# SebastianBitsch/SRGAN-ST

Hardware: AMD Instinct MI355X
Metric: HR images/sec (96px x4, B=16/GPU) G+D+ST-loss step (higher is better)
Workload: dtype f32; 1 GPU; srgan_x4_hr96_b16_G+D+ST-loss step: adv+mse+st, D updated every step (train.py:116-164; BASELINE metric); global_batch=16, hr=96, lr=24, parallelism=dp1, hip_graph=True, d_update_interval=1, d_sr_forward=run: all three discriminator forwards of train.py:136,155,158

## Files before the change

include/srganst.h:

```cpp
#ifndef SRGANST_H
#define SRGANST_H
#include <stdint.h>
#ifdef __cplusplus
extern "C" {
#endif

const char* sst_last_error(void);
int sst_version(void);
const char* sst_arch(void);
int sst_clear_error(void);
int sst_reload_env(void);

int sst_st_loss_workspace(int B, int H, int W, int64_t* partial_floats);
int sst_st_loss_fwd(const float* sr, const float* gt, float* loss, float* gS, float* partials,
                    unsigned* counter, int B, int H, int W, float sigma, float rho, int normalize,
                    void* stream);
int sst_st_loss_bwd(const float* sr, const float* gS, float* dsr, const float* scale_dev,
                    float scale_host, int accumulate, int B, int H, int W, float sigma, float rho,
                    void* stream);
int sst_st_maps_workspace(int B, int H, int W, int64_t* tile_floats);
int sst_st_maps(const float* x, const float* gt, float* Sx, float* Sgt, float* Fx, float* Fgt, float* d, float* tile_sums,
                int B, int H, int W, float sigma, float rho, int normalize, void* stream);
int sst_st_pixel_loss_fwd(const float* sr, const float* gt, float* loss, float* gS, float* partials, unsigned* counter,
                          float* pix_loss, float* pix_partials, int pix_mode, int B, int H, int W, float sigma, float rho,
                          int normalize, void* stream);
int sst_st_pixel_loss_bwd(const float* sr, const float* gt, const float* gS, float* dsr, const float* scale_dev, float scale_host,
                          float pix_weight, int pix_mode, int accumulate, int B, int H, int W, float sigma, float rho,
                          void* stream);

int64_t sst_conv_packed_floats(int Cout, int Cin, int ksize);
int sst_conv_pack(const float* w, float* wp, int Cout, int Cin, int ksize, int mode, void* stream);
int sst_conv_pack_multi(const void* jobs, int njobs, int total_blocks, void* stream);
int sst_conv_mtiles(int B, int Ho, int Wo);
int sst_conv_stat_tiles(int B, int H, int W, int Cin, int Cout, int ksize, int stride);
const char* sst_conv_kernel_name(int B, int H, int W, int Cin, int Cout, int ksize, int stride, int out_mode, int fused_in);
const char* sst_conv_wgrad_kernel_name(int B, int H, int W, int Cin, int Cout, int ksize, int stride, int njobs);
long sst_debug_big_tile_launches(void);
long sst_debug_band_launches(void);
long sst_debug_wgrad_band_launches(void);
int sst_debug_mfma_peak(float* out, int blocks, int iters, void* stream);
int sst_debug_bf16x3(const float* A, const float* B, float* C32, float* C3, int K, int mode, int blocks, void* stream);
int sst_debug_stamp(unsigned long long* out, int slot, void* stream);
int sst_conv_fwd(const float* x, const float* wp, float* y, float* y_pre, const float* bias,
                 const float* in_scale, const float* in_shift, const float* in_slope,
                 float in_slope_const, int in_act, const float* residual, float* stats,
                 float* stats_cnt, int out_mode, int B, int H, int W, int Cin, int Cout, int ksize,
                 int stride, void* stream);
int sst_conv_pipe_supported(int B, int H, int W, int Cin, int Cout, int ksize, int stride);
int sst_conv_pipe_stat_tiles(int B, int H, int W, int Cin, int Cout, int ksize, int stride);
int64_t sst_conv_pipe_ws_floats(int B, int H, int W, int Cin, int Cout, int ksize, int stride);
int sst_conv_pipe_fwd(const float* x, const float* wp, float* y, const float* bias, const float* in_scale,
                      const float* in_shift, const float* in_slope, float in_slope_const, int in_act, float* stats,
                      float* stats_cnt, const float* epi_y, const float* epi_scale, const float* epi_shift,
                      const float* epi_slope, float epi_slope_const, int epi_act, float* epi_partial, float* ws, int B,
                      int H, int W, int Cin, int Cout, int ksize, int stride, void* stream);
int sst_conv_pipe_groups_ok(int B, int H, int W, int Cin, int Cout, int ksize, int stride, int grp_images);
int sst_conv_pipe_fwd_grp(const float* x, const float* wp, float* y, const float* bias, const float* in_scale,
                          const float* in_shift, const float* in_slope, float in_slope_const, int in_act, float* stats,
                          float* stats_cnt, const float* epi_y, const float* epi_scale, const float* epi_shift,
                          const float* epi_slope, float epi_slope_const, int epi_act, float* epi_partial, float* ws, int B,
                          int H, int W, int Cin, int Cout, int ksize, int stride, int grp_images, void* stream);
int sst_conv_ns_supported(int B, int H, int W, int Cin, int Cout, int ksize, int stride, int out_mode);
int sst_conv_ns_fwd(const float* x, const float* wp, float* y, const float* bias, const float* in_scale,
                    const float* in_shift, const float* in_slope, float in_slope_const, int in_act, float* stats,
                    float* stats_cnt, const float* epi_y, const float* epi_scale, const float* epi_shift,
                    const float* epi_slope, float epi_slope_const, int epi_act, float* epi_partial, int B, int H, int W,
                    int Cin, int Cout, int ksize, int stride, int out_mode, int grp_images, void* stream);
int sst_conv_s2_dgrad_pipe_supported(int B, int H, int W, int Cin, int Cout);
int64_t sst_conv_s2_dgrad_pipe_ws_floats(int B, int H, int W, int Cin, int Cout);
int sst_conv_s2_dgrad_pipe(const float* dy, const float* wp, float* dx, float* ws, int B, int H, int W, int Cin, int Cout,
                           void* stream);
int sst_conv_s2_dgrad_pipe_stat_tiles(int B, int H, int W, int Cin, int Cout);
int sst_conv_s2_dgrad_pipe_bwdstats(const float* dy, const float* wp, float* dx, float* ws, const float* epi_y,
                                    const float* epi_scale, const float* epi_shift, const float* epi_slope,
                                    float epi_slope_const, int epi_act, float* epi_partial, int B, int H, int W, int Cin,
                                    int Cout, void* stream);
int sst_conv_s2_dgrad_pipe_groups_ok(int B, int H, int W, int Cin, int Cout, int grp_images);
int sst_conv_s2_dgrad_pipe_bwdstats_grp(const float* dy, const float* wp, float* dx, float* ws, const float* epi_y,
                                    const float* epi_scale, const float* epi_shift, const float* epi_slope,
                                    float epi_slope_const, int epi_act, float* epi_partial, int B, int H, int W, int Cin,
                                    int Cout, int grp_images, void* stream);
int sst_conv_dgrad_bwdstats(const float* x, const float* wp, float* y, const float* residual, const float* epi_y,
                            const float* epi_scale, const float* epi_shift, const float* epi_slope,
// ... 184 lines not shown
```

srgan-st_amd/csrc/conv_pipe.hip:

```cpp
#include "conv_common.h"
#include <cstdlib>
#include <type_traits>
#include "conv_epilogue.h"

int sst_conv_band_rows(int B, int H, int W, int Cin, int Cout, int ksize, int stride);

namespace {

constexpr int PIPE_RING = 9;

struct PipeArgs {
  const float* x;
  const float* wp;
  float* y;
  const float* bias;
  const float* in_scale; const float* in_shift; const float* in_slope; float in_slope_const; int in_act;
  float* stats; float* stats_cnt;
  const float* epi_y; const float* epi_scale; const float* epi_shift; const float* epi_slope;
  float epi_slope_const; int epi_act; float* epi_partial;
  float* ws;
  int B, H, W, Cin, Cout, Ho, Wo;
  int R;
  int tiles_x, n_mt, nfc, total_tiles, ncb, ksplit, cb_per, units;
#ifdef SST_PIPE_ABLATE
  int dbg;
#endif
  int gB, grows;
};

template <int S, int TW, int MODE>
struct PipeGeom {
  static constexpr int TH = 32 / TW;
  static constexpr int NB = TW == 2 ? 3 : 1;
  static constexpr int KSPAN = MODE ? 2 : 3;
  static constexpr int PW = (TW - 1) * S + KSPAN;
  static constexpr int PR = (TH - 1) * S + KSPAN + NB;
  static constexpr int NP = PW * PR;
  static constexpr int NU = (NP + 15) / 16;
  static constexpr int PS = 20;
  static constexpr int WAVE_FLOATS = NP * PS;
  static constexpr int NACC = MODE ? 4 : 1;
  static constexpr int NPAIR = MODE ? 2 : 1;
  static constexpr int SCRATCH = NPAIR * 4 * 32 * 33;
};
constexpr int S2D_CLS[9] = {0, 1, 1, 2, 2, 3, 3, 3, 3};
constexpr int S2D_TAP[9] = {0, 0, 1, 0, 1, 0, 1, 2, 3};

struct Stage {
  int b0, rem0, ix0, c0;
  int gin;
  const float* w;
};

#define PIPE_GLOAD(dst, voff, sbase) \
  asm volatile("s_nop 4\n\tglobal_load_dwordx4 %0, %1, %2" : "=v"(dst) : "v"(voff), "s"(sbase))
#define PIPE_WAIT(reg, n) asm volatile("s_waitcnt vmcnt(%1)" : "+v"(reg) : "n"(n))

__device__ __forceinline__ float half_sum(float t) {
  auto ror = [](float x, auto ctrl) {
    return __builtin_bit_cast(float, __builtin_amdgcn_update_dpp(0, __builtin_bit_cast(int, x), decltype(ctrl)::value, 0xf, 0xf, false));
  };
  t += ror(t, std::integral_constant<int, 0x128>{});
  t += ror(t, std::integral_constant<int, 0x124>{});
  t += ror(t, std::integral_constant<int, 0x122>{});
  t += ror(t, std::integral_constant<int, 0x121>{});
  t += __shfl_xor(t, 16, 64);
  return t;
}

template <int TW, int MODE = 0>
__device__ __forceinline__ void pipe_epilogue(const PipeArgs& a, float v[4], int r0, int ox0, int c0, int mt, int lane, bool first,
                                              int cls = 0) {
  constexpr int TH = 32 / TW;
  const int px = lane & 31;
  const int r = r0 + px / TW, ox = ox0 + px % TW;
  const bool pix_ok = r < a.R && ox < a.Wo;
  size_t obase;
  if (MODE) {
    obase = ((size_t)(2 * r + (cls >> 1)) * (2 * a.Wo) + 2 * ox + (cls & 1)) * a.Cout + c0;
    if (pix_ok) *reinterpret_cast<f32x4*>(a.y + obase) = f32x4{v[0], v[1], v[2], v[3]};
  }
  if (!MODE && a.bias) {
    const f32x4 bv = *reinterpret_cast<const f32x4*>(a.bias + c0);
#pragma unroll
    for (int j = 0; j < 4; ++j) v[j] += bv[j];
  }
  if (!MODE) {
    obase = ((size_t)r * a.Wo + ox) * a.Cout + c0;
    if (pix_ok) *reinterpret_cast<f32x4*>(a.y + obase) = f32x4{v[0], v[1], v[2], v[3]};
// ... 17 lines not shown
    }
  }
  if (a.epi_partial) {
    const float eslope = a.epi_slope ? a.epi_slope[0] : a.epi_slope_const;
    f32x4 yv = {0.f, 0.f, 0.f, 0.f}, es = {1.f, 1.f, 1.f, 1.f}, eh = {0.f, 0.f, 0.f, 0.f};
    if (pix_ok) yv = *reinterpret_cast<const f32x4*>(a.epi_y + obase);
    if (a.epi_scale) {
      const int ge = a.gB ? (r0 / a.grows) * a.Cout : 0;
      es = *reinterpret_cast<const f32x4*>(a.epi_scale + ge + c0);
      eh = *reinterpret_cast<const f32x4*>(a.epi_shift + ge + c0);
    }
    f32x4 q[3];
#pragma unroll
    for (int j = 0; j < 4; ++j) {
      const float g = pix_ok ? v[j] : 0.f;
      const float z = a.epi_scale ? fmaf(yv[j], es[j], eh[j]) : yv[j];
      float gz = g, q2 = 0.f;
      if (a.epi_act) {
        q2 = g * fminf(z, 0.f);
        gz = z > 0.f ? g : g * eslope;
      }
      q[0][j] = half_sum(gz);
      q[1][j] = half_sum(gz * yv[j]);
      q[2][j] = half_sum(q2);
    }
    if (px == 0) {
      const size_t prow = MODE ? (size_t)mt * 4 + cls : (size_t)mt;
#pragma unroll
      for (int k = 0; k < 3; ++k) *reinterpret_cast<f32x4*>(a.epi_partial + (prow * 3 + k) * a.Cout + c0) = q[k];
    }
  }
}

template <int S, int TW, int MODE, bool MS>
__global__ __launch_bounds__(CONV_NT, (S == 1 && MODE == 0 ? 3 : 2)) void conv_pipe_kernel(PipeArgs a) {
  using G = PipeGeom<S, TW, MODE>;
  constexpr int NACC = G::NACC, NPAIR = G::NPAIR;
  constexpr int PW = G::PW, NP = G::NP, NU = G::NU, NB = G::NB;
  constexpr int PS = G::PS;
  __shared__ __attribute__((aligned(16))) float patch[4 * G::WAVE_FLOATS];
  __shared__ __attribute__((aligned(16))) float scratch[G::SCRATCH];
  const int tid = threadIdx.x, wave = __builtin_amdgcn_readfirstlane(tid >> 6), lane = tid & 63;
  const int li = lane & 31, lh = lane >> 5;
  const int nwg = gridDim.x;
  const int HV = a.H + 1;
  const float slope = a.in_slope ? a.in_slope[0] : a.in_slope_const;
  const int c4 = wave * 16 + (lane & 3) * 4;
  const int p0 = lane >> 2;
  float* const lds = patch + wave * G::WAVE_FLOATS;

  int q = blockIdx.x;
  if (q >= a.units) return;
  int mt, nf, r0, ox0, oy0, cb, cb_end;
  Stage cur, nxt;
  auto decode = [&](int qq, int& mt_, int& nf_, int& ksi_, int& r0_, int& ox0_, int& b0_, int& oy0_) {
    mt_ = qq % a.n_mt;
    const int rest = qq / a.n_mt;
    nf_ = rest % a.nfc;
    ksi_ = rest / a.nfc;
    const int ty = mt_ / a.tiles_x, tx = mt_ - ty * a.tiles_x;
    r0_ = ty * G::TH;
    ox0_ = tx * TW;
    b0_ = r0_ / a.Ho;
    oy0_ = r0_ - b0_ * a.Ho;
  };
  auto make_stage = [&](int b0_, int oy0_, int ox0_, int nf_, int cb_) {
    Stage s;
    s.b0 = b0_;
    s.rem0 = oy0_ * S;
    s.ix0 = ox0_ * S - (MODE ? 0 : 1);
    s.c0 = cb_ * CB;
    s.gin = a.gB ? (b0_ / a.gB) * a.Cin : 0;
    s.w = a.wp + ((size_t)(nf_ * a.ncb + cb_) * 9 * 8) * 256 + wave * 512;
    return s;
  };
  int ksi, b0;
  decode(q, mt, nf, ksi, r0, ox0, b0, oy0);
  cb = ksi * a.cb_per;
  cb_end = cb + a.cb_per;
  cur = make_stage(b0, oy0, ox0, nf, cb);

  constexpr int NS = NU + 2;
  f32x4 sv[NU];
  unsigned okmask = 0;
  f32x4 ssc, ssh;
  const float* sc_base = a.in_scale ? a.in_scale : a.x;
  const float* sh_base = a.in_scale ? a.in_shift : a.x;
  unsigned boffs[MS ? NU : 1];
  auto stage_load = [&](const Stage& s, bool same_tile) {
#ifdef SST_PIPE_ABLATE
    if (a.dbg & 4) return;
#endif
    if (MS && same_tile) {
#pragma unroll
      for (int u = 0; u < NU; ++u) {
        boffs[u] += CB * 4u;
        PIPE_GLOAD(sv[u], boffs[u], a.x);
      }
    } else {
      okmask = 0;
#pragma unroll
      for (int u = 0; u < NU; ++u) {
        const int p = p0 + 16 * u;
        const int pr = p / PW, pc = p - pr * PW;
        int rr = s.rem0 + pr, b = s.b0;
#pragma unroll
        for (int k = 0; k <= NB; ++k) {
          const bool wrap = rr >= HV;
          rr -= wrap ? HV : 0;
          b += wrap ? 1 : 0;
        }
        const int iy = MODE ? rr : rr - 1, ix = s.ix0 + pc;
        const bool ok = p < NP && (MODE ? rr < a.H : rr >= 1) && b < a.B && (unsigned)ix < (unsigned)a.W;
        const int off = ((b * a.H + iy) * a.W + ix) * a.Cin + s.c0 + c4;
        const unsigned boff = (ok ? (unsigned)off : (unsigned)c4) * 4u;
        if (MS) boffs[u] = boff;
        PIPE_GLOAD(sv[u], boff, a.x);
        okmask |= ok ? (1u << u) : 0u;
      }
    }
    const unsigned coff = (unsigned)(a.in_scale ? s.gin + s.c0 + c4 : c4) * 4u;
    PIPE_GLOAD(ssc, coff, sc_base);
    PIPE_GLOAD(ssh, coff, sh_base);
  };
  auto stage_store = [&]() {
#ifdef SST_PIPE_ABLATE
    if (a.dbg & 1) return;
#endif
#pragma unroll
    for (int u = 0; u < NU; ++u) {
      const int p = p0 + 16 * u;
      if (p >= NP) continue;
      f32x4 t = sv[u];
      if (a.in_scale) {
#pragma unroll
        for (int j = 0; j < 4; ++j) t[j] = fmaf(t[j], ssc[j], ssh[j]);
      }
      if (a.in_act == ACT_SLOPE) {
#pragma unroll
        for (int j = 0; j < 4; ++j) t[j] = t[j] > 0.f ? t[j] : t[j] * slope;
      }
      if (!((okmask >> u) & 1u)) t = f32x4{0.f, 0.f, 0.f, 0.f};
      *reinterpret_cast<f32x4*>(&lds[p * PS + (lane & 3) * 4]) = t;
    }
  };

  auto lane_base = [&](int oy0_) {
    const int tr = li / TW, tc = li - tr * TW;
    int cross = 0;
#pragma unroll
    for (int k = 1; k <= NB; ++k) cross += (oy0_ + tr >= k * a.Ho) ? 1 : 0;
    return ((S * tr + cross) * PW + tc * S) * PS + 4 * lh;
  };
  int a_base = lane_base(oy0);

  f32x4 ring[PIPE_RING];
  const unsigned wlane = lane * 16u;
#define PIPE_WCHUNK(dst, w, i) PIPE_GLOAD(dst, wlane, (w) + (((i) >> 1) * 8 + ((i) & 1)) * 256)

#pragma unroll
  for (int i = 0; i < PIPE_RING; ++i) PIPE_WCHUNK(ring[i], cur.w, i);
  stage_load(cur, false);
  asm volatile("s_waitcnt vmcnt(0)" ::: "memory");
  __builtin_amdgcn_sched_barrier(0);
  stage_store();

  f32x16 acc[NACC];
#pragma unroll
  for (int k = 0; k < NACC; ++k)
#pragma unroll
    for (int r = 0; r < 16; ++r) acc[k][r] = 0.f;

  for (;;) {
    const bool unit_end = cb + 1 == cb_end;
    int n_q = q, n_mt = mt, n_nf = nf, n_r0 = r0, n_ox0 = ox0, n_oy0 = oy0, n_cb = cb + 1, n_cb_end = cb_end;
    bool more = true;
    if (unit_end) {
      n_q = q + nwg;
      more = n_q < a.units;
      if (more) {
        int n_ksi, n_b0;
        decode(n_q, n_mt, n_nf, n_ksi, n_r0, n_ox0, n_b0, n_oy0);
        n_cb = n_ksi * a.cb_per;
        n_cb_end = n_cb + a.cb_per;
        nxt = make_stage(n_b0, n_oy0, n_ox0, n_nf, n_cb);
      } else {
        nxt = cur;
      }
    } else {
      nxt = cur;
      nxt.c0 += CB;
      nxt.w += (size_t)9 * 8 * 256;
    }

    {
      const float* ab = lds + a_base;
      f32x4 av = *reinterpret_cast<const f32x4*>(ab);
      __builtin_amdgcn_sched_barrier(0);
#pragma unroll
      for (int i = 0; i < 18; ++i) {
        f32x4 an = av;
        if (i + 1 < 18) {
          const int t = (i + 1) >> 1;
          const int ntx = MODE ? 1 + (S2D_CLS[t] & 1) : 3, tt = MODE ? S2D_TAP[t] : t;
          an = *reinterpret_cast<const f32x4*>(ab + ((tt / ntx) * PW + (tt % ntx)) * PS + ((i + 1) & 1) * 8);
        }
        if (i == 0 || i >= 10) PIPE_WAIT(ring[i % PIPE_RING], 8); else PIPE_WAIT(ring[i % PIPE_RING], 8 + NS);
        const f32x4 bv = ring[i % PIPE_RING];
        constexpr int dummy_ = 0;
        (void)dummy_;
        const int ai = MODE ? S2D_CLS[i >> 1] : 0;
#ifdef SST_PIPE_ABLATE
        if (!(a.dbg & 16))
#endif
#pragma unroll
        for (int j = 0; j < 4; ++j) acc[ai] = __builtin_amdgcn_mfma_f32_32x32x2f32(av[j], bv[j], acc[ai], 0, 0, 0);
#ifdef SST_PIPE_ABLATE
        if (a.dbg & 8) { PIPE_GLOAD(ring[i % PIPE_RING], wlane, a.wp); } else
#endif
        if (i + PIPE_RING < 18) PIPE_WCHUNK(ring[i % PIPE_RING], cur.w, i + PIPE_RING);
        else PIPE_WCHUNK(ring[i % PIPE_RING], nxt.w, i + PIPE_RING - 18);
        if (i == 0) stage_load(nxt, !unit_end);
        av = an;
        __builtin_amdgcn_sched_barrier(0);
      }
    }
#ifdef SST_PIPE_ABLATE
    if (unit_end && (a.dbg & 2)) {
      if (acc[0][0] == 12345.f) a.y[0] = acc[0][0];
      if (!more) return;
      a_base = lane_base(n_oy0);
    } else
#endif
    if (unit_end) {
      const int cl = 8 * wave + 4 * lh;
#pragma unroll
      for (int k0 = 0; k0 < NACC; k0 += NPAIR) {
        __syncthreads();
#pragma unroll
        for (int k = 0; k < NPAIR; ++k)
#pragma unroll
          for (int r = 0; r < 16; ++r) {
            const int row = (r & 3) + 8 * (r >> 2) + 4 * lh;
            scratch[((k * 4 + wave) * 32 + row) * 33 + li] = acc[k0 + k][r];
            acc[k0 + k][r] = 0.f;
          }
        __syncthreads();
#pragma unroll
        for (int k = 0; k < NPAIR; ++k) {
          float v[4];
#pragma unroll
          for (int j = 0; j < 4; ++j) {
            float t = scratch[((k * 4 + 0) * 32 + li) * 33 + cl + j];
            t += scratch[((k * 4 + 1) * 32 + li) * 33 + cl + j];
            t += scratch[((k * 4 + 2) * 32 + li) * 33 + cl + j];
            t += scratch[((k * 4 + 3) * 32 + li) * 33 + cl + j];
            v[j] = t;
          }
          if (a.ksplit > 1) {
            const int tile = nf * a.n_mt + mt;
            const int part = cb / a.cb_per;
            *reinterpret_cast<f32x4*>(a.ws + (((size_t)part * a.total_tiles + tile) * NACC + k0 + k) * 1024 + li * 32 + cl) =
                f32x4{v[0], v[1], v[2], v[3]};
          } else {
            pipe_epilogue<TW, MODE>(a, v, r0, ox0, nf * 32 + cl, mt, lane, nf == 0 && wave == 0, k0 + k);
          }
        }
      }
      if (!more) return;
      a_base = lane_base(n_oy0);
    }
    stage_store();
    q = n_q; mt = n_mt; nf = n_nf; r0 = n_r0; ox0 = n_ox0; oy0 = n_oy0; cb = n_cb; cb_end = n_cb_end;
    cur = nxt;
  }
}

template <int TW, int MODE>
__global__ __launch_bounds__(CONV_NT) void pipe_reduce_kernel(PipeArgs a) {
  constexpr int NACC = MODE ? 4 : 1;
  const int tid = threadIdx.x, wave = tid >> 6, lane = tid & 63;
  const int tile = blockIdx.x / NACC, cls = blockIdx.x - tile * NACC;
  const int nf = tile / a.n_mt, mt = tile - nf * a.n_mt;
  const int ty = mt / a.tiles_x, tx = mt - ty * a.tiles_x;
  const int li = lane & 31, cl = 8 * wave + 4 * (lane >> 5);
  const size_t slab = (size_t)a.total_tiles * NACC * 1024;
  const float* src = a.ws + ((size_t)tile * NACC + cls) * 1024 + li * 32 + cl;
  f32x4 s = *reinterpret_cast<const f32x4*>(src);
  for (int k = 1; k < a.ksplit; ++k) {
    const f32x4 t = *reinterpret_cast<const f32x4*>(src + k * slab);
#pragma unroll
    for (int j = 0; j < 4; ++j) s[j] += t[j];
  }
  float v[4] = {s[0], s[1], s[2], s[3]};
  pipe_epilogue<TW, MODE>(a, v, ty * (32 / TW), tx * TW, nf * 32 + cl, mt, lane, nf == 0 && wave == 0, cls);
}

struct PipePlan {
  int tw;
  int ksplit, n_mt, tiles_x, nfc, ncb;
};

PipePlan pipe_plan(int B, int H, int W, int Cin, int Cout, int ksize, int stride) {
  PipePlan pl{};
  if (ksize != 3 || (stride != 1 && stride != 2) || (Cin % 64) || (Cout % 32) || B <= 0) return pl;
  if (stride == 2 && ((H | W) & 1)) return pl;
  if (Cout <= 64 && sst_conv_band_rows(B, H, W, Cin, Cout, ksize, stride)) return pl;
  const int Ho = (H - 1) / stride + 1, Wo = (W - 1) / stride + 1;
  int tw = 0;
  if (Wo % 8 == 0 && Ho >= 3) tw = 8;
  else if (Wo % 4 == 0 && Ho >= 7) tw = 4;
  else if (Wo % 2 == 0 && Ho >= 5) tw = 2;
  if (!tw) return pl;
  const int th = 32 / tw;
  pl.tiles_x = Wo / tw;
  pl.n_mt = pl.tiles_x * ((B * Ho + th - 1) / th);
  pl.nfc = Cout / 32;
  pl.ncb = Cin / 64;
  const long tiles = (long)pl.n_mt * pl.nfc;
  int maxks = 1;
  while (maxks < 4 && pl.ncb % (maxks * 2) == 0) maxks *= 2;
  if (tiles * maxks < 256) return pl;
  int ks = 1;
  while (tiles * ks < 1024 && ks < maxks) ks *= 2;
  pl.ksplit = ks;
  pl.tw = tw;
  return pl;
}

constexpr int PIPE_CUS = 256;

}

SST_API int sst_conv_pipe_supported(int B, int H, int W, int Cin, int Cout, int ksize, int stride) {
  return pipe_plan(B, H, W, Cin, Cout, ksize, stride).tw;
}
SST_API int sst_conv_pipe_stat_tiles(int B, int H, int W, int Cin, int Cout, int ksize, int stride) {
  return pipe_plan(B, H, W, Cin, Cout, ksize, stride).n_mt;
}
SST_API int64_t sst_conv_pipe_ws_floats(int B, int H, int W, int Cin, int Cout, int ksize, int stride) {
  const PipePlan pl = pipe_plan(B, H, W, Cin, Cout, ksize, stride);
  return (pl.tw && pl.ksplit > 1) ? (int64_t)pl.ksplit * pl.n_mt * pl.nfc * 1024 : 0;
}

SST_API int sst_conv_pipe_groups_ok(int B, int H, int W, int Cin, int Cout, int ksize, int stride, int grp_images) {
  const PipePlan pl = pipe_plan(B, H, W, Cin, Cout, ksize, stride);
  if (!pl.tw || grp_images <= 0 || B % grp_images) return 0;
  const int Ho = (H - 1) / stride + 1;
  return (grp_images * Ho) % (32 / pl.tw) == 0;
}

SST_API int sst_conv_pipe_fwd_grp(const float* x, const float* wp, float* y, const float* bias, const float* in_scale,
                                  const float* in_shift, const float* in_slope, float in_slope_const, int in_act, float* stats,
                                  float* stats_cnt, const float* epi_y, const float* epi_scale, const float* epi_shift,
                                  const float* epi_slope, float epi_slope_const, int epi_act, float* epi_partial, float* ws, int B,
                                  int H, int W, int Cin, int Cout, int ksize, int stride, int grp_images, void* stream) {
  SST_REQUIRE(x && wp && y, "sst_conv_pipe_fwd: null pointer");
  const PipePlan pl = pipe_plan(B, H, W, Cin, Cout, ksize, stride);
  SST_REQUIRE(grp_images == 0 || grp_images == B || sst_conv_pipe_groups_ok(B, H, W, Cin, Cout, ksize, stride, grp_images),
              "sst_conv_pipe_fwd: coefficient groups of %d images do not end on tile boundaries (B=%d H=%d W=%d stride=%d)", grp_images, B,
              H, W, stride);
  SST_REQUIRE(pl.tw, "sst_conv_pipe_fwd: shape B=%d H=%d W=%d Cin=%d Cout=%d k=%d stride=%d is not taken by the pipelined kernel", B,
              H, W, Cin, Cout, ksize, stride);
  SST_REQUIRE((in_scale == nullptr) == (in_shift == nullptr), "sst_conv_pipe_fwd: in_scale/in_shift must come together");
  SST_REQUIRE(!stats || stats_cnt, "sst_conv_pipe_fwd: stats needs stats_cnt");
  SST_REQUIRE(!epi_partial || (epi_y && !stats && ((epi_scale == nullptr) == (epi_shift == nullptr))),
              "sst_conv_pipe_fwd: backward partials need epi_y and exclude forward stats");
  SST_REQUIRE(pl.ksplit == 1 || ws, "sst_conv_pipe_fwd: this shape splits K over workgroups and needs the workspace");
  SST_REQUIRE((int64_t)B * H * W * Cin < (1ll << 29), "sst_conv_pipe_fwd: input too large for 32-bit byte offsets");
  PipeArgs a;
  a.x = x; a.wp = wp; a.y = y; a.bias = bias; a.in_scale = in_scale; a.in_shift = in_shift; a.in_slope = in_slope;
  a.in_slope_const = in_slope_const; a.in_act = in_act; a.stats = stats; a.stats_cnt = stats_cnt;
  a.epi_y = epi_y; a.epi_scale = epi_scale; a.epi_shift = epi_shift; a.epi_slope = epi_slope; a.epi_slope_const = epi_slope_const;
  a.epi_act = epi_act; a.epi_partial = epi_partial; a.ws = ws;
  a.B = B; a.H = H; a.W = W; a.Cin = Cin; a.Cout = Cout;
  a.Ho = (H - 1) / stride + 1; a.Wo = (W - 1) / stride + 1; a.R = B * a.Ho;
  a.tiles_x = pl.tiles_x; a.n_mt = pl.n_mt; a.nfc = pl.nfc; a.total_tiles = pl.n_mt * pl.nfc; a.ncb = pl.ncb;
  a.ksplit = pl.ksplit; a.cb_per = pl.ncb / pl.ksplit; a.units = a.total_tiles * pl.ksplit;
  a.gB = (grp_images > 0 && grp_images < B) ? grp_images : 0;
  a.grows = a.gB * a.Ho;
#ifdef SST_PIPE_ABLATE
  a.dbg = sst_env("SST_PIPE_DBG") ? atoi(sst_env("SST_PIPE_DBG")) : 0;
#endif
  int wg_per_cu = stride == 1 ? 3 : 2;
  if (const char* e = sst_env("SST_PIPE_GPC")) {
    const int v = atoi(e);
    if (v >= 1 && v < wg_per_cu) wg_per_cu = v;
  }
  const int grid = a.units < wg_per_cu * PIPE_CUS ? a.units : wg_per_cu * PIPE_CUS;
  hipStream_t st = sst_stream(stream);
#define SST_PIPE_LAUNCH(S_, TW_)                                                                  \
  do {                                                                                            \
    if (a.cb_per > 1) conv_pipe_kernel<S_, TW_, 0, true><<<grid, CONV_NT, 0, st>>>(a);            \
    else conv_pipe_kernel<S_, TW_, 0, false><<<grid, CONV_NT, 0, st>>>(a);                        \
    SST_LAUNCH_CHECK("conv_pipe_kernel");                                                         \
    if (pl.ksplit > 1) {                                                                          \
      pipe_reduce_kernel<TW_, 0><<<a.total_tiles, CONV_NT, 0, st>>>(a);                           \
      SST_LAUNCH_CHECK("pipe_reduce_kernel");                                                     \
    }                                                                                             \
  } while (0)
  if (stride == 1) {
    if (pl.tw == 8) SST_PIPE_LAUNCH(1, 8); else if (pl.tw == 4) SST_PIPE_LAUNCH(1, 4); else SST_PIPE_LAUNCH(1, 2);
  } else {
    if (pl.tw == 8) SST_PIPE_LAUNCH(2, 8); else if (pl.tw == 4) SST_PIPE_LAUNCH(2, 4); else SST_PIPE_LAUNCH(2, 2);
  }
#undef SST_PIPE_LAUNCH
  return SST_OK;
}

SST_API int sst_conv_pipe_fwd(const float* x, const float* wp, float* y, const float* bias, const float* in_scale,
                              const float* in_shift, const float* in_slope, float in_slope_const, int in_act, float* stats,
                              float* stats_cnt, const float* epi_y, const float* epi_scale, const float* epi_shift,
                              const float* epi_slope, float epi_slope_const, int epi_act, float* epi_partial, float* ws, int B,
                              int H, int W, int Cin, int Cout, int ksize, int stride, void* stream) {
  return sst_conv_pipe_fwd_grp(x, wp, y, bias, in_scale, in_shift, in_slope, in_slope_const, in_act, stats, stats_cnt, epi_y, epi_scale,
                               epi_shift, epi_slope, epi_slope_const, epi_act, epi_partial, ws, B, H, W, Cin, Cout, ksize, stride, 0, stream);
}

int64_t sst_conv_s2_dgrad_pipe_section(int Cout, int Cin);
SST_API int sst_conv_s2_dgrad_pipe_bwdstats_grp(const float* dy, const float* wp, float* dx, float* ws, const float* epi_y,
                                                const float* epi_scale, const float* epi_shift, const float* epi_slope,
                                                float epi_slope_const, int epi_act, float* epi_partial, int B, int H, int W, int Cin,
                                                int Cout, int grp_images, void* stream);

namespace {
PipePlan pipe_plan_s2d(int B, int H, int W, int Cin, int Cout) {
// ... 92 lines not shown
```

srgan-st_amd/srganst/_abi.py:

```python
from __future__ import annotations

import ctypes
import os
from ctypes import c_char_p, c_float, c_int, c_int64, c_void_p, POINTER

_HERE = os.path.dirname(os.path.abspath(__file__))
LIB_PATH = os.environ.get("SST_LIB_PATH") or os.path.join(_HERE, "lib", "libsrganst.so")

P = c_void_p

SIGNATURES = {
    "sst_last_error": (c_char_p, []),
    "sst_version": (c_int, []),
    "sst_arch": (c_char_p, []),
    "sst_clear_error": (c_int, []),
    "sst_reload_env": (c_int, []),
    "sst_st_loss_workspace": (c_int, [c_int, c_int, c_int, POINTER(c_int64)]),
    "sst_st_loss_fwd": (c_int, [P, P, P, P, P, P, c_int, c_int, c_int, c_float, c_float, c_int, P]),
    "sst_st_loss_bwd": (c_int, [P, P, P, P, c_float, c_int, c_int, c_int, c_int, c_float, c_float, P]),
    "sst_st_pixel_loss_fwd": (c_int, [P, P, P, P, P, P, P, P, c_int, c_int, c_int, c_int, c_float, c_float, c_int, P]),
    "sst_st_pixel_loss_bwd": (c_int, [P, P, P, P, P, c_float, c_float, c_int, c_int, c_int, c_int, c_int, c_float, c_float, P]),
    "sst_st_maps_workspace": (c_int, [c_int, c_int, c_int, POINTER(c_int64)]),
    "sst_st_maps": (c_int, [P, P, P, P, P, P, P, P, c_int, c_int, c_int, c_float, c_float, c_int, P]),
    "sst_conv_packed_floats": (c_int64, [c_int, c_int, c_int]),
    "sst_conv_pack": (c_int, [P, P, c_int, c_int, c_int, c_int, P]),
    "sst_conv_pack_multi": (c_int, [P, c_int, c_int, P]),
    "sst_conv_kernel_name": (c_char_p, [c_int, c_int, c_int, c_int, c_int, c_int, c_int, c_int, c_int]),
    "sst_conv_wgrad_kernel_name": (c_char_p, [c_int, c_int, c_int, c_int, c_int, c_int, c_int, c_int]),
    "sst_debug_big_tile_launches": (ctypes.c_long, []),
    "sst_adam_flat": (c_int, [P, P, P, P, c_int64, P, P, c_int, ctypes.c_double, ctypes.c_double, ctypes.c_double,
                            ctypes.c_double, P]),
    "sst_debug_band_launches": (ctypes.c_long, []),
    "sst_debug_wgrad_band_launches": (ctypes.c_long, []),
    "sst_debug_mfma_peak": (c_int, [P, c_int, c_int, P]),
    "sst_debug_bf16x3": (c_int, [P, P, P, P, c_int, c_int, c_int, P]),
    "sst_debug_stamp": (c_int, [P, c_int, P]),
    "sst_conv_mtiles": (c_int, [c_int, c_int, c_int]),
    "sst_conv_stat_tiles": (c_int, [c_int, c_int, c_int, c_int, c_int, c_int, c_int]),
    "sst_conv_fwd": (c_int, [P, P, P, P, P, P, P, P, c_float, c_int, P, P, P, c_int,
                             c_int, c_int, c_int, c_int, c_int, c_int, c_int, P]),
    "sst_conv_pipe_supported": (c_int, [c_int, c_int, c_int, c_int, c_int, c_int, c_int]),
    "sst_conv_pipe_stat_tiles": (c_int, [c_int, c_int, c_int, c_int, c_int, c_int, c_int]),
    "sst_conv_pipe_ws_floats": (c_int64, [c_int, c_int, c_int, c_int, c_int, c_int, c_int]),
    "sst_conv_pipe_fwd": (c_int, [P, P, P, P, P, P, P, c_float, c_int, P, P, P, P, P, P, c_float, c_int, P, P,
                                  c_int, c_int, c_int, c_int, c_int, c_int, c_int, P]),
    "sst_conv_pipe_groups_ok": (c_int, [c_int, c_int, c_int, c_int, c_int, c_int, c_int, c_int]),
    "sst_conv_pipe_fwd_grp": (c_int, [P, P, P, P, P, P, P, c_float, c_int, P, P, P, P, P, P, c_float, c_int, P, P,
                                      c_int, c_int, c_int, c_int, c_int, c_int, c_int, c_int, P]),
    "sst_conv_ns_supported": (c_int, [c_int, c_int, c_int, c_int, c_int, c_int, c_int, c_int]),
    "sst_conv_ns_fwd": (c_int, [P, P, P, P, P, P, P, c_float, c_int, P, P, P, P, P, P, c_float, c_int, P,
                                c_int, c_int, c_int, c_int, c_int, c_int, c_int, c_int, c_int, P]),
    "sst_conv_s2_dgrad_pipe_supported": (c_int, [c_int, c_int, c_int, c_int, c_int]),
    "sst_conv_s2_dgrad_pipe_ws_floats": (c_int64, [c_int, c_int, c_int, c_int, c_int]),
    "sst_conv_s2_dgrad_pipe": (c_int, [P, P, P, P, c_int, c_int, c_int, c_int, c_int, P]),
    "sst_conv_s2_dgrad_pipe_stat_tiles": (c_int, [c_int, c_int, c_int, c_int, c_int]),
    "sst_conv_s2_dgrad_pipe_bwdstats": (c_int, [P, P, P, P, P, P, P, P, c_float, c_int, P, c_int, c_int, c_int, c_int, c_int, P]),
    "sst_conv_s2_dgrad_pipe_groups_ok": (c_int, [c_int, c_int, c_int, c_int, c_int, c_int]),
    "sst_conv_s2_dgrad_pipe_bwdstats_grp": (c_int, [P, P, P, P, P, P, P, P, c_float, c_int, P, c_int, c_int, c_int, c_int, c_int, c_int, P]),
    "sst_conv_acc_supported": (c_int, [c_int, c_int, c_int, c_int, c_int, c_int, c_int]),
    "sst_conv_fwd_acc": (c_int, [P, P, P, P, P, P, P, P, c_float, c_int, P, P, P, c_float, c_float, c_float, P, P, P, P, P, P, P,
                                 c_int, c_int, c_int, c_int, c_int, c_int, c_int, P]),
    "sst_conv_dgrad_fused_acc": (c_int, [P, P, P, P, P, c_float, c_int, P, P, P, P, P, P, P, P, c_float, c_int, P, P, P, P, c_float, P, P, P,
                                         P, c_int, c_int, c_int, c_int, c_int, c_int, c_int, P]),
    "sst_bn_finalize_acc": (c_int, [P, c_int, c_int, c_float, P, P, P, P, P, P, P, P, c_float, c_float, P]),
    "sst_conv_fwd_resin": (c_int, [P, P, P, P, P, P, P, P, P, P, P, c_int, c_int, c_int, c_int, c_int, c_int, P]),
    "sst_conv_dgrad_bwdstats": (c_int, [P, P, P, P, P, P, P, P, c_float, c_int, P, c_int, c_int, c_int, c_int, c_int, c_int, P]),
    "sst_conv_dgrad_fused": (c_int, [P, P, P, P, P, P, P, P, c_float, c_int, P, P, P, P, P, P, P, P, c_float, c_int, P,
                                     c_int, c_int, c_int, c_int, c_int, c_int, P]),
    "sst_conv_wgrad_chunks": (c_int, [c_int, c_int, c_int, c_int, c_int, c_int]),
    "sst_conv_wgrad_chunks2": (c_int, [c_int, c_int, c_int, c_int, c_int, c_int, c_int, c_int]),
    "sst_conv_wgrad": (c_int, [P, P, P, P, P, P, P, c_float, c_int, c_int, c_int, c_int, c_int, c_int,
                               c_int, c_int, c_int, P]),
    "sst_conv_wgrad_groups_ok": (c_int, [c_int, c_int, c_int, c_int, c_int, c_int, c_int, c_int]),
    "sst_conv_wgrad_grp": (c_int, [P, P, P, P, P, P, P, c_float, c_int, c_int, c_int, c_int, c_int, c_int,
                                   c_int, c_int, c_int, c_int, P]),
    "sst_conv_wgrad_grouped": (c_int, [P, c_int, c_int, c_int, c_int, c_int, c_int, c_int, c_int, c_int, P]),
# ... 120 lines not shown
```

Before: 3262 HR images/s.

## Pair adjacent output-channel blocks in stride-2 pipelined conv to reuse input patches

Adds 'pair units' to the stride-2 forward pipelined conv kernel. One workgroup computes two adjacent 32-channel output blocks, sharing the LDS input patch and A operands while streaming two weight rings with a smaller ring depth. A host-side makespan model picks how many channel pairs to form so that fewer, heavier units fill the 256-CU grid better. This trades extra registers and lower occupancy risk, plus a more complex wait and epilogue path, for less input reload and better wave quantization.

Result: no change. 3267 HR images/s, median of 6 (+0.2%).

```diff
diff --git a/include/srganst.h b/include/srganst.h
--- a/include/srganst.h
+++ b/include/srganst.h
@@ -49,6 +49,7 @@
 int sst_conv_pipe_supported(int B, int H, int W, int Cin, int Cout, int ksize, int stride);
 int sst_conv_pipe_stat_tiles(int B, int H, int W, int Cin, int Cout, int ksize, int stride);
 int64_t sst_conv_pipe_ws_floats(int B, int H, int W, int Cin, int Cout, int ksize, int stride);
+int sst_conv_pipe_pair_units(int B, int H, int W, int Cin, int Cout, int ksize, int stride, int* pairs, int* singles);
 int sst_conv_pipe_fwd(const float* x, const float* wp, float* y, const float* bias, const float* in_scale,
                       const float* in_shift, const float* in_slope, float in_slope_const, int in_act, float* stats,
                       float* stats_cnt, const float* epi_y, const float* epi_scale, const float* epi_shift,
diff --git a/srgan-st_amd/csrc/conv_pipe.hip b/srgan-st_amd/csrc/conv_pipe.hip
--- a/srgan-st_amd/csrc/conv_pipe.hip
+++ b/srgan-st_amd/csrc/conv_pipe.hip
@@ -8,6 +8,7 @@
 namespace {
 
 constexpr int PIPE_RING = 9;
+constexpr int PIPE_RING_PAIR = 6;
 
 struct PipeArgs {
   const float* x;
@@ -26,6 +27,7 @@
   int dbg;
 #endif
   int gB, grows;
+  int npair, pair_units;
 };
 
 template <int S, int TW, int MODE>
@@ -55,6 +57,7 @@
 #define PIPE_GLOAD(dst, voff, sbase) \
   asm volatile("s_nop 4\n\tglobal_load_dwordx4 %0, %1, %2" : "=v"(dst) : "v"(voff), "s"(sbase))
 #define PIPE_WAIT(reg, n) asm volatile("s_waitcnt vmcnt(%1)" : "+v"(reg) : "n"(n))
+#define PIPE_WAIT2(reg, reg2, n) asm volatile("s_waitcnt vmcnt(%2)" : "+v"(reg), "+v"(reg2) : "n"(n))
 
 __device__ __forceinline__ float half_sum(float t) {
   auto ror = [](float x, auto ctrl) {
@@ -138,8 +141,9 @@
   }
 }
 
-template <int S, int TW, int MODE, bool MS>
+template <int S, int TW, int MODE, bool MS, bool PAIRS = false>
 __global__ __launch_bounds__(CONV_NT, (S == 1 && MODE == 0 ? 3 : 2)) void conv_pipe_kernel(PipeArgs a) {
+  static_assert(!PAIRS || (S == 2 && MODE == 0), "pair units: stride-2 forward only");
   using G = PipeGeom<S, TW, MODE>;
   constexpr int NACC = G::NACC, NPAIR = G::NPAIR;
   constexpr int PW = G::PW, NP = G::NP, NU = G::NU, NB = G::NB;
@@ -151,19 +155,32 @@
   const int nwg = gridDim.x;
   const int HV = a.H + 1;
   const float slope = a.in_slope ? a.in_slope[0] : a.in_slope_const;
-  const int c4 = wave * 16 + (lane & 3) * 4;
+  const int c4_ = wave * 16 + (lane & 3) * 4;
   const int p0 = lane >> 2;
   float* const lds = patch + wave * G::WAVE_FLOATS;
 
   int q = blockIdx.x;
   if (q >= a.units) return;
   int mt, nf, r0, ox0, oy0, cb, cb_end;
+  bool pair = false;
   Stage cur, nxt;
-  auto decode = [&](int qq, int& mt_, int& nf_, int& ksi_, int& r0_, int& ox0_, int& b0_, int& oy0_) {
-    mt_ = qq % a.n_mt;
-    const int rest = qq / a.n_mt;
-    nf_ = rest % a.nfc;
-    ksi_ = rest / a.nfc;
+  auto decode = [&](int qq, int& mt_, int& nf_, int& ksi_, int& r0_, int& ox0_, int& b0_, int& oy0_, bool& pair_) {
+    if constexpr (PAIRS) {
+      pair_ = qq < a.pair_units;
+      const int slots = pair_ ? a.npair : a.nfc - 2 * a.npair;
+      if (!pair_) qq -= a.pair_units;
+      mt_ = qq % a.n_mt;
+      const int rest = qq / a.n_mt;
+      const int slot = rest % slots;
+      nf_ = pair_ ? 2 * slot : 2 * a.npair + slot;
+      ksi_ = rest / slots;
+    } else {
+      pair_ = false;
+      mt_ = qq % a.n_mt;
+      const int rest = qq / a.n_mt;
+      nf_ = rest % a.nfc;
+      ksi_ = rest / a.nfc;
+    }
     const int ty = mt_ / a.tiles_x, tx = mt_ - ty * a.tiles_x;
     r0_ = ty * G::TH;
     ox0_ = tx * TW;
@@ -181,10 +198,13 @@
     return s;
   };
   int ksi, b0;
-  decode(q, mt, nf, ksi, r0, ox0, b0, oy0);
+  decode(q, mt, nf, ksi, r0, ox0, b0, oy0, pair);
   cb = ksi * a.cb_per;
   cb_end = cb + a.cb_per;
   cur = make_stage(b0, oy0, ox0, nf, cb);
+  const size_t wblk2 = (size_t)a.ncb * 72 * 256;
+  const float* cur_w2 = cur.w + (pair ? wblk2 : 0);
+  const float* nxt_w2 = cur_w2;
 
   constexpr int NS = NU + 2;
   f32x4 sv[NU];
@@ -193,7 +213,7 @@
   const float* sc_base = a.in_scale ? a.in_scale : a.x;
   const float* sh_base = a.in_scale ? a.in_shift : a.x;
   unsigned boffs[MS ? NU : 1];
-  auto stage_load = [&](const Stage& s, bool same_tile) {
+  auto stage_load = [&](const Stage& s, bool same_tile) __attribute__((always_inline)) {
 #ifdef SST_PIPE_ABLATE
     if (a.dbg & 4) return;
 #endif
@@ -205,10 +225,20 @@
       }
     } else {
       okmask = 0;
+      int p0v = p0, c4 = c4_;
+      if constexpr (PAIRS) asm volatile("" : "+v"(p0v), "+v"(c4));
+      int pr_u = p0v / PW, pc_u = p0v - pr_u * PW;
 #pragma unroll
       for (int u = 0; u < NU; ++u) {
-        const int p = p0 + 16 * u;
-        const int pr = p / PW, pc = p - pr * PW;
+        const int p = p0v + 16 * u;
+        int pr, pc;
+        if constexpr (PAIRS) {
+          pr = pr_u; pc = pc_u;
+          pc_u += 16 % PW; pr_u += 16 / PW;
+          if (pc_u >= PW) { pc_u -= PW; ++pr_u; }
+        } else {
+          pr = p / PW; pc = p - pr * PW;
+        }
         int rr = s.rem0 + pr, b = s.b0;
 #pragma unroll
         for (int k = 0; k <= NB; ++k) {
@@ -225,11 +255,11 @@
         okmask |= ok ? (1u << u) : 0u;
       }
     }
-    const unsigned coff = (unsigned)(a.in_scale ? s.gin + s.c0 + c4 : c4) * 4u;
+    const unsigned coff = (unsigned)(a.in_scale ? s.gin + s.c0 + c4_ : c4_) * 4u;
     PIPE_GLOAD(ssc, coff, sc_base);
     PIPE_GLOAD(ssh, coff, sh_base);
   };
-  auto stage_store = [&]() {
+  auto stage_store = [&]() __attribute__((always_inline)) {
 #ifdef SST_PIPE_ABLATE
     if (a.dbg & 1) return;
 #endif
@@ -252,132 +282,117 @@
   };
 
   auto lane_base = [&](int oy0_) {
-    const int tr = li / TW, tc = li - tr * TW;
+    int li_b = li, lh_b = lh;
+    if constexpr (PAIRS) {
+      int lane_b = lane;
+      asm volatile("" : "+v"(lane_b));
+      li_b = lane_b & 31; lh_b = lane_b >> 5;
+    }
+    const int tr = li_b / TW, tc = li_b - tr * TW;
     int cross = 0;
 #pragma unroll
     for (int k = 1; k <= NB; ++k) cross += (oy0_ + tr >= k * a.Ho) ? 1 : 0;
-    return ((S * tr + cross) * PW + tc * S) * PS + 4 * lh;
+    return ((S * tr + cross) * PW + tc * S) * PS + 4 * lh_b;
   };
   int a_base = lane_base(oy0);
 
-  f32x4 ring[PIPE_RING];
+  constexpr int RING = PAIRS ? PIPE_RING_PAIR : PIPE_RING;
+  static_assert(18 % RING == 0, "a stage's 18 chunks must fill the ring a whole number of times");
+  f32x4 ring[RING];
+  f32x4 ring2[PAIRS ? RING : 1];
   const unsigned wlane = lane * 16u;
 #define PIPE_WCHUNK(dst, w, i) PIPE_GLOAD(dst, wlane, (w) + (((i) >> 1) * 8 + ((i) & 1)) * 256)
 
 #pragma unroll
-  for (int i = 0; i < PIPE_RING; ++i) PIPE_WCHUNK(ring[i], cur.w, i);
+  for (int i = 0; i < RING; ++i) PIPE_WCHUNK(ring[i], cur.w, i);
+  if constexpr (PAIRS) {
+    if (pair) {
+#pragma unroll
+      for (int i = 0; i < RING; ++i) PIPE_WCHUNK(ring2[i], cur_w2, i);
+    } else {
+#pragma unroll
+      for (int i = 0; i < RING; ++i) ring2[i] = f32x4{0.f, 0.f, 0.f, 0.f};
+    }
+  }
   stage_load(cur, false);
   asm volatile("s_waitcnt vmcnt(0)" ::: "memory");
   __builtin_amdgcn_sched_barrier(0);
   stage_store();
 
-  f32x16 acc[NACC];
-#pragma unroll
-  for (int k = 0; k < NACC; ++k)
+  constexpr int NACC2 = PAIRS ? 2 : NACC;
+  f32x16 acc[NACC2];
+#pragma unroll
+  for (int k = 0; k < NACC2; ++k)
 #pragma unroll
     for (int r = 0; r < 16; ++r) acc[k][r] = 0.f;
 
   for (;;) {
     const bool unit_end = cb + 1 == cb_end;
     int n_q = q, n_mt = mt, n_nf = nf, n_r0 = r0, n_ox0 = ox0, n_oy0 = oy0, n_cb = cb + 1, n_cb_end = cb_end;
-    bool more = true;
+    bool more = true, n_pair = pair;
     if (unit_end) {
       n_q = q + nwg;
       more = n_q < a.units;
       if (more) {
         int n_ksi, n_b0;
-        decode(n_q, n_mt, n_nf, n_ksi, n_r0, n_ox0, n_b0, n_oy0);
+        decode(n_q, n_mt, n_nf, n_ksi, n_r0, n_ox0, n_b0, n_oy0, n_pair);
         n_cb = n_ksi * a.cb_per;
         n_cb_end = n_cb + a.cb_per;
         nxt = make_stage(n_b0, n_oy0, n_ox0, n_nf, n_cb);
       } else {
         nxt = cur;
       }
+      if constexpr (PAIRS) nxt_w2 = nxt.w + (more && n_pair ? wblk2 : 0);
     } else {
       nxt = cur;
       nxt.c0 += CB;
       nxt.w += (size_t)9 * 8 * 256;
-    }
-
+      if constexpr (PAIRS) nxt_w2 = cur_w2 + (size_t)9 * 8 * 256;
+    }
+
+#define PIPE_SECTION_KLOOP
     {
-      const float* ab = lds + a_base;
-      f32x4 av = *reinterpret_cast<const f32x4*>(ab);
-      __builtin_amdgcn_sched_barrier(0);
-#pragma unroll
-      for (int i = 0; i < 18; ++i) {
-        f32x4 an = av;
-        if (i + 1 < 18) {
-          const int t = (i + 1) >> 1;
-          const int ntx = MODE ? 1 + (S2D_CLS[t] & 1) : 3, tt = MODE ? S2D_TAP[t] : t;
-          an = *reinterpret_cast<const f32x4*>(ab + ((tt / ntx) * PW + (tt % ntx)) * PS + ((i + 1) & 1) * 8);
-        }
-        if (i == 0 || i >= 10) PIPE_WAIT(ring[i % PIPE_RING], 8); else PIPE_WAIT(ring[i % PIPE_RING], 8 + NS);
-        const f32x4 bv = ring[i % PIPE_RING];
-        constexpr int dummy_ = 0;
-        (void)dummy_;
-        const int ai = MODE ? S2D_CLS[i >> 1] : 0;
-#ifdef SST_PIPE_ABLATE
-        if (!(a.dbg & 16))
-#endif
-#pragma unroll
-        for (int j = 0; j < 4; ++j) acc[ai] = __builtin_amdgcn_mfma_f32_32x32x2f32(av[j], bv[j], acc[ai], 0, 0, 0);
-#ifdef SST_PIPE_ABLATE
-        if (a.dbg & 8) { PIPE_GLOAD(ring[i % PIPE_RING], wlane, a.wp); } else
-#endif
-        if (i + PIPE_RING < 18) PIPE_WCHUNK(ring[i % PIPE_RING], cur.w, i + PIPE_RING);
-        else PIPE_WCHUNK(ring[i % PIPE_RING], nxt.w, i + PIPE_RING - 18);
-        if (i == 0) stage_load(nxt, !unit_end);
-        av = an;
-        __builtin_amdgcn_sched_barrier(0);
-      }
-    }
+      bool pair_unit = false;
+      if constexpr (PAIRS) pair_unit = pair;
+#include "conv_pipe_unit.h"
+    }
+#undef PIPE_SECTION_KLOOP
+
 #ifdef SST_PIPE_ABLATE
     if (unit_end && (a.dbg & 2)) {
-      if (acc[0][0] == 12345.f) a.y[0] = acc[0][0];
+      if (acc[0][0] == 12345.f || acc[NACC2 - 1][0] == 12345.f) a.y[0] = acc[0][0];
       if (!more) return;
       a_base = lane_base(n_oy0);
     } else
 #endif
     if (unit_end) {
-      const int cl = 8 * wave + 4 * lh;
-#pragma unroll
-      for (int k0 = 0; k0 < NACC; k0 += NPAIR) {
-        __syncthreads();
-#pragma unroll
-        for (int k = 0; k < NPAIR; ++k)
-#pragma unroll
-          for (int r = 0; r < 16; ++r) {
-            const int row = (r & 3) + 8 * (r >> 2) + 4 * lh;
-            scratch[((k * 4 + wave) * 32 + row) * 33 + li] = acc[k0 + k][r];
-            acc[k0 + k][r] = 0.f;
-          }
-        __syncthreads();
-#pragma unroll
-        for (int k = 0; k < NPAIR; ++k) {
-          float v[4];
-#pragma unroll
-          for (int j = 0; j < 4; ++j) {
-            float t = scratch[((k * 4 + 0) * 32 + li) * 33 + cl + j];
-            t += scratch[((k * 4 + 1) * 32 + li) * 33 + cl + j];
-            t += scratch[((k * 4 + 2) * 32 + li) * 33 + cl + j];
-            t += scratch[((k * 4 + 3) * 32 + li) * 33 + cl + j];
-            v[j] = t;
-          }
-          if (a.ksplit > 1) {
-            const int tile = nf * a.n_mt + mt;
-            const int part = cb / a.cb_per;
-            *reinterpret_cast<f32x4*>(a.ws + (((size_t)part * a.total_tiles + tile) * NACC + k0 + k) * 1024 + li * 32 + cl) =
-                f32x4{v[0], v[1], v[2], v[3]};
-          } else {
-            pipe_epilogue<TW, MODE>(a, v, r0, ox0, nf * 32 + cl, mt, lane, nf == 0 && wave == 0, k0 + k);
-          }
+      int li_e = li, lh_e = lh, lane_e = lane;
+      if constexpr (PAIRS) {
+        asm volatile("" : "+v"(lane_e));
+        li_e = lane_e & 31; lh_e = lane_e >> 5;
+      }
+      const int cl = 8 * wave + 4 * lh_e;
+#define PIPE_SECTION_EXCHANGE
+#define PIPE_BLK 0
+#include "conv_pipe_unit.h"
+#undef PIPE_BLK
+      if constexpr (PAIRS) {
+        if (pair) {
+#define PIPE_BLK 1
+#include "conv_pipe_unit.h"
+#undef PIPE_BLK
         }
       }
+#undef PIPE_SECTION_EXCHANGE
       if (!more) return;
       a_base = lane_base(n_oy0);
     }
+    if constexpr (PAIRS) {
+      if (pair && !n_pair) asm volatile("s_waitcnt vmcnt(0)" ::: "memory");
+      cur_w2 = nxt_w2;
+    }
     stage_store();
-    q = n_q; mt = n_mt; nf = n_nf; r0 = n_r0; ox0 = n_ox0; oy0 = n_oy0; cb = n_cb; cb_end = n_cb_end;
+    q = n_q; mt = n_mt; nf = n_nf; r0 = n_r0; ox0 = n_ox0; oy0 = n_oy0; cb = n_cb; cb_end = n_cb_end; pair = n_pair;
     cur = nxt;
   }
 }
@@ -402,10 +417,38 @@
   pipe_epilogue<TW, MODE>(a, v, ty * (32 / TW), tx * TW, nf * 32 + cl, mt, lane, nf == 0 && wave == 0, cls);
 }
 
+constexpr int PIPE_CUS = 256;
+
 struct PipePlan {
   int tw;
   int ksplit, n_mt, tiles_x, nfc, ncb;
+  int npair;
 };
+
+inline double pipe_pair_c2(int tw, bool multi_stage) { return tw == 8 ? (multi_stage ? 2.0 : 1.753) : tw == 4 ? 2.025 : 2.010; }
+
+inline double pipe_makespan(long blocks, long pairs, double c2) {
+  const long units = blocks - pairs;
+  const long grid = units < 2 * PIPE_CUS ? units : 2 * PIPE_CUS;
+  return (double)((units + grid - 1) / grid) + (double)((pairs + grid - 1) / grid) * (c2 - 1.0);
+}
+
+int pipe_plan_pairs(const PipePlan& pl) {
+  const char* e = sst_env("SST_PIPE_PAIR");
+  const int mode = e ? atoi(e) : 1;
+  if (mode == 0 || pl.nfc < 2) return 0;
+  if (mode == 2) return pl.nfc / 2;
+  if (mode > 2) return mode - 3 < pl.nfc / 2 ? mode - 3 : pl.nfc / 2;
+  const long per = (long)pl.n_mt * pl.ksplit, blocks = per * pl.nfc;
+  const double c2 = pipe_pair_c2(pl.tw, pl.ncb / pl.ksplit > 1);
+  int best = 0;
+  double best_t = pipe_makespan(blocks, 0, c2) - 1e-9;
+  for (int np = 1; np <= pl.nfc / 2; ++np) {
+    const double t = pipe_makespan(blocks, per * np, c2);
+    if (t <= best_t) { best = np; best_t = t; }
+  }
+  return best;
+}
 
 PipePlan pipe_plan(int B, int H, int W, int Cin, int Cout, int ksize, int stride) {
   PipePlan pl{};
@@ -431,10 +474,10 @@
   while (tiles * ks < 1024 && ks < maxks) ks *= 2;
   pl.ksplit = ks;
   pl.tw = tw;
+  if (stride == 2) pl.npair = pipe_plan_pairs(pl);
   return pl;
 }
 
-constexpr int PIPE_CUS = 256;
 
 }
 
@@ -447,6 +490,13 @@
 SST_API int64_t sst_conv_pipe_ws_floats(int B, int H, int W, int Cin, int Cout, int ksize, int stride) {
   const PipePlan pl = pipe_plan(B, H, W, Cin, Cout, ksize, stride);
   return (pl.tw && pl.ksplit > 1) ? (int64_t)pl.ksplit * pl.n_mt * pl.nfc * 1024 : 0;
+}
+SST_API int sst_conv_pipe_pair_units(int B, int H, int W, int Cin, int Cout, int ksize, int stride, int* pairs, int* singles) {
+  SST_REQUIRE(pairs && singles, "sst_conv_pipe_pair_units: null pointer");
+  const PipePlan pl = pipe_plan(B, H, W, Cin, Cout, ksize, stride);
+  *pairs = pl.tw ? pl.npair * pl.n_mt * pl.ksplit : 0;
+  *singles = pl.tw ? (pl.nfc - 2 * pl.npair) * pl.n_mt * pl.ksplit : 0;
+  return SST_OK;
 }
 
 SST_API int sst_conv_pipe_groups_ok(int B, int H, int W, int Cin, int Cout, int ksize, int stride, int grp_images) {
@@ -482,7 +532,9 @@
   a.B = B; a.H = H; a.W = W; a.Cin = Cin; a.Cout = Cout;
   a.Ho = (H - 1) / stride + 1; a.Wo = (W - 1) / stride + 1; a.R = B * a.Ho;
   a.tiles_x = pl.tiles_x; a.n_mt = pl.n_mt; a.nfc = pl.nfc; a.total_tiles = pl.n_mt * pl.nfc; a.ncb = pl.ncb;
-  a.ksplit = pl.ksplit; a.cb_per = pl.ncb / pl.ksplit; a.units = a.total_tiles * pl.ksplit;
+  a.ksplit = pl.ksplit; a.cb_per = pl.ncb / pl.ksplit;
+  a.npair = pl.npair; a.pair_units = pl.npair * pl.n_mt * pl.ksplit;
+  a.units = a.total_tiles * pl.ksplit - a.pair_units;
   a.gB = (grp_images > 0 && grp_images < B) ? grp_images : 0;
   a.grows = a.gB * a.Ho;
 #ifdef SST_PIPE_ABLATE
@@ -497,7 +549,10 @@
   hipStream_t st = sst_stream(stream);
 #define SST_PIPE_LAUNCH(S_, TW_)                                                                  \
   do {                                                                                            \
-    if (a.cb_per > 1) conv_pipe_kernel<S_, TW_, 0, true><<<grid, CONV_NT, 0, st>>>(a);            \
+    if (S_ == 2 && a.npair > 0) {                                                                 \
+      if (a.cb_per > 1) conv_pipe_kernel<2, TW_, 0, true, true><<<grid, CONV_NT, 0, st>>>(a);            \
+      else conv_pipe_kernel<2, TW_, 0, false, true><<<grid, CONV_NT, 0, st>>>(a);                        \
+    } else if (a.cb_per > 1) conv_pipe_kernel<S_, TW_, 0, true><<<grid, CONV_NT, 0, st>>>(a);     \
     else conv_pipe_kernel<S_, TW_, 0, false><<<grid, CONV_NT, 0, st>>>(a);                        \
     SST_LAUNCH_CHECK("conv_pipe_kernel");                                                         \
     if (pl.ksplit > 1) {                                                                          \
diff --git a/srgan-st_amd/csrc/conv_pipe_unit.h b/srgan-st_amd/csrc/conv_pipe_unit.h
--- /dev/null
+++ b/srgan-st_amd/csrc/conv_pipe_unit.h
@@ -0,0 +1,91 @@
+#if defined(PIPE_SECTION_KLOOP)
+{
+    constexpr int WV = RING - 1;
+    const float* ab = lds + a_base;
+    f32x4 av = *reinterpret_cast<const f32x4*>(ab);
+    __builtin_amdgcn_sched_barrier(0);
+#pragma unroll
+    for (int i = 0; i < 18; ++i) {
+      f32x4 an = av;
+      if (i + 1 < 18) {
+        const int t = (i + 1) >> 1;
+        const int ntx = MODE ? 1 + (S2D_CLS[t] & 1) : 3, tt = MODE ? S2D_TAP[t] : t;
+        an = *reinterpret_cast<const f32x4*>(ab + ((tt / ntx) * PW + (tt % ntx)) * PS + ((i + 1) & 1) * 8);
+      }
+      if (pair_unit) {
+        if (i == 0 || i > RING) PIPE_WAIT2(ring[i % RING], ring2[PAIRS ? i % RING : 0], 2 * WV);
+        else PIPE_WAIT2(ring[i % RING], ring2[PAIRS ? i % RING : 0], 2 * WV + NS);
+      } else {
+        if (i == 0 || i > RING) PIPE_WAIT(ring[i % RING], WV); else PIPE_WAIT(ring[i % RING], WV + NS);
+      }
+      const f32x4 bv = ring[i % RING];
+      constexpr int dummy_ = 0;
+      (void)dummy_;
+      const int ai = MODE ? S2D_CLS[i >> 1] : 0;
+#ifdef SST_PIPE_ABLATE
+      if (!(a.dbg & 16))
+#endif
+      {
+#pragma unroll
+        for (int j = 0; j < 4; ++j) acc[ai] = __builtin_amdgcn_mfma_f32_32x32x2f32(av[j], bv[j], acc[ai], 0, 0, 0);
+        if (pair_unit) {
+          const f32x4 bv2 = ring2[PAIRS ? i % RING : 0];
+#pragma unroll
+          for (int j = 0; j < 4; ++j) acc[NACC2 - 1] = __builtin_amdgcn_mfma_f32_32x32x2f32(av[j], bv2[j], acc[NACC2 - 1], 0, 0, 0);
+        }
+      }
+#ifdef SST_PIPE_ABLATE
+      if (a.dbg & 8) {
+        PIPE_GLOAD(ring[i % RING], wlane, a.wp);
+        if (pair_unit) PIPE_GLOAD(ring2[PAIRS ? i % RING : 0], wlane, a.wp);
+      } else
+#endif
+      if (i + RING < 18) {
+        PIPE_WCHUNK(ring[i % RING], cur.w, i + RING);
+        if (pair_unit) PIPE_WCHUNK(ring2[PAIRS ? i % RING : 0], cur_w2, i + RING);
+      } else {
+        PIPE_WCHUNK(ring[i % RING], nxt.w, i + RING - 18);
+        if (pair_unit) PIPE_WCHUNK(ring2[PAIRS ? i % RING : 0], nxt_w2, i + RING - 18);
+      }
+      if (i == 0) stage_load(nxt, !unit_end);
+      av = an;
+      __builtin_amdgcn_sched_barrier(0);
+    }
+}
+#elif defined(PIPE_SECTION_EXCHANGE)
+{
+#pragma unroll
+    for (int k0 = 0; k0 < NACC; k0 += NPAIR) {
+      __syncthreads();
+#pragma unroll
+      for (int k = 0; k < NPAIR; ++k)
+#pragma unroll
+        for (int r = 0; r < 16; ++r) {
+          const int row = (r & 3) + 8 * (r >> 2) + 4 * lh_e;
+          scratch[((k * 4 + wave) * 32 + row) * 33 + li_e] = acc[PIPE_BLK * NACC + k0 + k][r];
+          acc[PIPE_BLK * NACC + k0 + k][r] = 0.f;
+        }
+      __syncthreads();
+#pragma unroll
+      for (int k = 0; k < NPAIR; ++k) {
+        float v[4];
+#pragma unroll
+        for (int j = 0; j < 4; ++j) {
+          float t = scratch[((k * 4 + 0) * 32 + li_e) * 33 + cl + j];
+          t += scratch[((k * 4 + 1) * 32 + li_e) * 33 + cl + j];
+          t += scratch[((k * 4 + 2) * 32 + li_e) * 33 + cl + j];
+          t += scratch[((k * 4 + 3) * 32 + li_e) * 33 + cl + j];
+          v[j] = t;
+        }
+        if (a.ksplit > 1) {
+          const int tile = (nf + PIPE_BLK) * a.n_mt + mt;
+          const int part = cb / a.cb_per;
+          *reinterpret_cast<f32x4*>(a.ws + (((size_t)part * a.total_tiles + tile) * NACC + k0 + k) * 1024 + li_e * 32 + cl) =
+              f32x4{v[0], v[1], v[2], v[3]};
+        } else {
+          pipe_epilogue<TW, MODE>(a, v, r0, ox0, (nf + PIPE_BLK) * 32 + cl, mt, lane_e, (nf + PIPE_BLK) == 0 && wave == 0, k0 + k);
+        }
+      }
+    }
+}
+#endif
diff --git a/srgan-st_amd/srganst/_abi.py b/srgan-st_amd/srganst/_abi.py
--- a/srgan-st_amd/srganst/_abi.py
+++ b/srgan-st_amd/srganst/_abi.py
@@ -42,6 +42,7 @@
     "sst_conv_pipe_supported": (c_int, [c_int, c_int, c_int, c_int, c_int, c_int, c_int]),
     "sst_conv_pipe_stat_tiles": (c_int, [c_int, c_int, c_int, c_int, c_int, c_int, c_int]),
     "sst_conv_pipe_ws_floats": (c_int64, [c_int, c_int, c_int, c_int, c_int, c_int, c_int]),
+    "sst_conv_pipe_pair_units": (c_int, [c_int, c_int, c_int, c_int, c_int, c_int, c_int, P, P]),
     "sst_conv_pipe_fwd": (c_int, [P, P, P, P, P, P, P, c_float, c_int, P, P, P, P, P, P, c_float, c_int, P, P,
                                   c_int, c_int, c_int, c_int, c_int, c_int, c_int, P]),
     "sst_conv_pipe_groups_ok": (c_int, [c_int, c_int, c_int, c_int, c_int, c_int, c_int, c_int]),
```
